# Gongzihang6/Pointcept-KeypointDetection

Hardware: AMD Instinct MI355X
Metric: Mpoints/sec PTv3 fwd @100k pts/scene, 1024-pt window; keypoint offset L2 vs ref (higher is better)
Workload: dtype bf16; 1 GPU; OffsetKeypointPTv3 (PT-v3m1 fork config, 46.2M params) eval forward, 1 x 100000-point synthetic surface scene(s) per GPU, patch 1024, serialization + sparse conv + attention + head included; points_per_gpu=100000, parallelism=replicas x1 (scene-sharded, no collective), forwards_in_flight=1

## Files before the change

### include/ptv3_hip.h

```cpp
#ifndef PTV3_HIP_H
#define PTV3_HIP_H
#include <stddef.h>
#include <stdint.h>

#ifdef __cplusplus
extern "C" {
#endif

#define PTV3_F32 0
#define PTV3_BF16 1

#define PTV3_OK 0
#define PTV3_ERR_ARG 1
#define PTV3_ERR_LAUNCH 2
#define PTV3_ERR_UNSUPPORTED 3

#define PTV3_ORDER_Z 0
#define PTV3_ORDER_Z_TRANS 1
#define PTV3_ORDER_HILBERT 2
#define PTV3_ORDER_HILBERT_TRANS 3

#define PTV3_ACT_NONE 0
#define PTV3_ACT_GELU 1
#define PTV3_ACT_RELU 2
// ... 125 lines not shown
                         const void* res, void* y, const float* gamma2, const float* beta2, void* y2, int64_t m, int c,
                         float eps, int dtype, void* stream);

int ptv3_affine_act(const void* x, const float* scale, const float* shift, int act, void* y, int64_t m,
                    int c, int dtype, void* stream);

int ptv3_cast(const void* x, int src_dtype, void* y, int dst_dtype, int64_t count, void* stream);

size_t ptv3_pool_workspace_bytes(int64_t n);
int ptv3_pool_segments(const int64_t* code0, const int64_t* order0, int64_t n, int shift_bits,
                       const int64_t* batch, int64_t* cluster, int32_t* seg_start, int32_t* n_out,
                       int64_t* pooled_offset, void* workspace, size_t workspace_bytes, void* stream);
int ptv3_pool_reduce(const void* feat, const float* coord, const int64_t* grid_coord,
                     const int64_t* batch, const int64_t* code, int k, const int64_t* order0,
                     const int32_t* seg_start, int64_t n, int64_t n_out, int c, int pooling_depth,
                     const float* bn_scale, const float* bn_shift, int act, const int* row_perm_host,
                     void* feat_out, float* coord_out, int64_t* grid_out, int64_t* batch_out,
                     int64_t* code_out, int dtype, void* stream);

typedef struct {
  int32_t dtype, in_channels , num_stages, num_orders;
  int32_t enc_depths[8], enc_channels[8], enc_heads[8], enc_patch[8];
  int32_t dec_depths[8], dec_channels[8], dec_heads[8], dec_patch[8];
  int32_t stride[8];
  int32_t enc_mode, enable_flash;
  int32_t head_hidden, head_out;
  float mlp_ratio, ln_eps, qk_scale ;
} ptv3_model_desc;

typedef struct {
  const void* grid_coord; int32_t coord_is_i64;
  const void* feat;
  const int64_t* batch;
  const int64_t* offset;
  const int64_t* offset_host;
  int32_t b; int64_t n;
  int32_t depth;
  const int32_t* order_ids_host;
  const int32_t* pool_perm_host;
  int64_t *code, *order, *inverse;
  void* out_feat;
  float* out_head;
  int64_t* stage_points_host;
  int32_t* depth_out;
  int64_t* batch_out;
  int32_t inputs_resident;
  int32_t overlap_calls;
  const void* raw_feat;
  int32_t raw_feat_channels;
  int32_t raw_feat_dtype;
  int64_t arena_n;
  int32_t arena_b;
  void* executor;
} ptv3_forward_io;

void* ptv3_executor_create(void);
int ptv3_executor_destroy(void* executor);

size_t ptv3_forward_workspace_bytes(const ptv3_model_desc* desc, int64_t n, int b);
int ptv3_forward(const ptv3_model_desc* desc, const void* const* params, int num_params,
                 const ptv3_forward_io* io, void* workspace, size_t workspace_bytes, void* stream);

size_t ptv3_gemm_tn_workspace_bytes(int64_t m, int cout, int cin, int kvol);
int ptv3_gemm_tn(const void* dy, const void* x, const int32_t* nbr, float* dw, float* dbias, int64_t m, int cout,
                 int cin, int kvol, int dtype, void* workspace, size_t workspace_bytes, void* stream);
size_t ptv3_col_reduce_workspace_bytes(int64_t m, int c);
int ptv3_col_reduce(const void* a, const void* b, const float* mu, const float* rs, float mu_scale, int mode, float* out,
                    int64_t m, int c, int dtype, void* workspace, size_t workspace_bytes, void* stream);
int ptv3_bn_finalize(const float* sum, const float* centred_sq, int64_t m, const float* weight, const float* bias,
                     float* running_mean, float* running_var, float momentum, float eps, float* mean, float* rstd,
                     float* scale, float* shift, int c, void* stream);
int ptv3_bn_bwd_coeffs(const float* sums, int64_t m, const float* weight, const float* rstd, const float* mean, float* ca,
                       float* cb, float* cc, int c, void* stream);
int ptv3_layernorm_bwd(const void* x, const void* dy, const void* add, const float* gamma, float eps, void* dx,
                       float* dgamma_dbeta, int64_t m, int c, int dtype, void* workspace,
                       size_t workspace_bytes, void* stream);
int ptv3_act_bwd(const void* dy, const void* x, const float* scale, const float* shift, int act, void* dx,
                 int64_t m, int c, int dtype, void* stream);
int ptv3_affine2(const void* dy, const void* x, const float* ca, const float* cb, const float* cc, void* dx,
                 int64_t m, int c, int dtype, void* stream);
int ptv3_pool_max_bwd(const void* feat, const void* dy, const int64_t* order0, const int32_t* seg_start,
                      int64_t n_out, int c, void* dfeat, int dtype, void* stream);
int ptv3_segment_sum(const void* dy, const int64_t* order0, const int32_t* seg_start, int64_t n_out, int c,
                     void* out, int dtype, void* stream);
size_t ptv3_window_attn_bwd_workspace_bytes(int64_t n, int64_t n_pad, int c, int heads, int dtype);
int ptv3_window_attn_bwd(const void* qkv, const void* out, const void* dout, const int32_t* win_order,
                         const int32_t* win_inverse, void* dqkv, int64_t n, int64_t n_pad, int c, int heads,
                         int patch, float scale, int dtype, void* workspace, size_t workspace_bytes,
                         void* stream);
int ptv3_window_attn_varlen_bwd(const void* qkv, const void* out, const void* dout, const int32_t* win_order,
                                const int32_t* win_inverse, const int32_t* cu_seqlens, int num_windows, void* dqkv,
                                int64_t n, int64_t n_pad, int c, int heads, int max_seqlen, float scale, int dtype,
                                void* workspace, size_t workspace_bytes, void* stream);
int ptv3_window_attn_train_fwd(const void* qkv, const int32_t* win_order, const int32_t* win_inverse,
                               const int32_t* cu_seqlens, int num_windows, void* out, float* lse, int64_t n,
                               int64_t n_pad, int c, int heads, int patch, float scale, double sum_len_sq, int dtype,
                               void* stream);
int ptv3_window_attn_train_bwd(const void* qkv, const void* out, const void* dout, const float* lse,
                               const int32_t* win_order, const int32_t* win_inverse, const int32_t* cu_seqlens,
                               int num_windows, void* dqkv, int64_t n, int64_t n_pad, int c, int heads, int patch,
                               float scale, int dtype, void* workspace, size_t workspace_bytes, void* stream);
int ptv3_window_attn_drop_fwd(const void* qkv, const int32_t* win_order, const int32_t* win_inverse,
                              const int32_t* cu_seqlens, int num_windows, void* out, int64_t n, int64_t n_pad, int c,
                              int heads, int patch, float scale, float p_drop, uint32_t seed, int dtype, void* stream);
int ptv3_window_attn_drop_bwd(const void* qkv, const void* out, const void* dout, const int32_t* win_order,
                              const int32_t* win_inverse, const int32_t* cu_seqlens, int num_windows, void* dqkv,
// ... 337 lines not shown
```

### pointcept-keypointdetection_amd/csrc/engine.hip

```cpp
#include <algorithm>
#include <chrono>
#include <mutex>
#include <stdio.h>
#include <stdlib.h>
#include <vector>
#include "common.h"
#include "window_attn.h"

namespace ptv3 {

struct Arena {
  char* base; size_t cap; size_t off; size_t peak; bool dry; bool failed;
  void* alloc(size_t bytes) {
    size_t a = (off + 255) / 256 * 256;
    off = a + bytes;
    if (off > peak) peak = off;
    if (dry) return (void*)(uintptr_t)256;
    if (off > cap) { failed = true; return nullptr; }
    return base + a;
  }
};

__global__ void make_indices_kernel(const int64_t* __restrict__ batch, const void* __restrict__ grid,
                                    int is_i64, int64_t n, int32_t* __restrict__ idx,
// ... 237 lines not shown
    RUN(ptv3_halo_plan_build(L.nbr3, L.row_order, L.n, L.halo, L.halo_bytes, sg));
    if (!dry && ok()) { L.halo_ready = X->event_at(40 + st); (void)hipEventRecord(L.halo_ready, sg); }
  }

  void conv3(Level& L, const void* w, void* out, int C, const float* bias, bool first_block) {
    if (L.halo && !first_block && ptv3_conv_halo_policy(L.n, C, C, 27, d->dtype)) {
      if (!dry && ok() && !L.halo_waited) { (void)hipStreamWaitEvent(sf, L.halo_ready, 0); L.halo_waited = true; }
      RUN(ptv3_conv_halo(L.conv_feat, w, out, L.n, C, L.nbr3, L.row_order, L.halo, L.halo_bytes, bias, nullptr, nullptr, 0,
                         nullptr, nullptr, nullptr, d->dtype, sf));
      return;
    }
    gemm(L.conv_feat, w, out, L.n, C, C, 27, L.nbr3, L.row_order, bias, nullptr, nullptr, 0, nullptr, nullptr, nullptr);
  }

  bool rows_path(int64_t n, int C, int hidden) const {
    static const int64_t min_rows = [] { const char* e = getenv("PTV3_ROWS_MIN"); return e ? atoll(e) : (int64_t)0; }();
    return n >= min_rows && ptv3_rows_linear_capable(C, 3 * C, d->dtype, n) && ptv3_rows_linear_capable(C, C, d->dtype, n) &&
           ptv3_rows_linear_capable(C, hidden, d->dtype, n);
  }

  int patch_K(const Level& L, int patch) const {
    if (d->enable_flash) return patch;
    int64_t mn = L.off_host[0];
    for (size_t i = 1; i < L.off_host.size(); ++i) mn = std::min(mn, L.off_host[i] - L.off_host[i - 1]);
    return (int)std::min<int64_t>(mn, patch);
  }

  void window_plan(Level& L, Plan& P, int K) {
    int64_t n_pad = 0, prev = 0;
    for (int64_t o : L.off_host) {
      int64_t cnt = o - prev;
      n_pad += cnt > K ? (cnt + K - 1) / K * K : cnt;
      prev = o;
    }
    P.K = K; P.n_pad = n_pad;
    bool ragged = false;
    P.nwin = 0; P.sum_len_sq = 0.0; prev = 0;
    for (int64_t o : L.off_host) {
      const int64_t cnt = o - prev;
      prev = o;
      P.nwin += (int)((cnt + K - 1) / K);
      if (cnt < K) { ragged = true; P.sum_len_sq += (double)cnt * cnt; }
      else P.sum_len_sq += (double)((cnt + K - 1) / K) * K * K;
    }
    const int k = d->num_orders;
    int32_t* wo = (int32_t*)G->alloc((size_t)k * n_pad * 4);
    int32_t* wi = (int32_t*)G->alloc((size_t)k * L.n * 4);
    P.cu = (ragged || (dry && d->enable_flash)) ? (int32_t*)G->alloc(((size_t)P.nwin + L.off_host.size() + 1) * 4) : nullptr;
    if (!ragged && !dry) P.cu = nullptr;
    RUN(ptv3_window_plan(L.order, L.inverse, L.offset, (int)L.off_host.size(), k, L.n, n_pad, K, wo, wi, P.cu, sg));
    for (int i = 0; i < k; ++i) { P.wo[i] = wo + (int64_t)i * n_pad; P.wi[i] = wi + (int64_t)i * L.n; }
  }

  hipEvent_t stem_ready = nullptr;
  void level0_sites(Level& L, const void* grid_in, int is_i64) {
    L.indices = (int32_t*)G->alloc((size_t)L.n * 16);
    L.row_order = (int32_t*)G->alloc((size_t)L.n * 4);
    int64_t* g64 = (int64_t*)G->alloc((size_t)L.n * 24);
    L.grid = g64;
    L.table_bytes = ptv3_subm_block_table_bytes(L.n);
    L.table = G->alloc(L.table_bytes);
    RUN(ptv3_subm_sites(L.batch, grid_in, is_i64, L.n, L.indices, g64, L.table, L.table_bytes, sg));
    RUN(ptv3_subm_build_block_table_zeroed(L.indices, L.n, L.table, L.table_bytes, sg));
    if (!dry && ok()) { stem_ready = X->event_at(19); (void)hipEventRecord(stem_ready, sg); }
  }

  void level_tables(Level& L, int st) {
    L.nbr3 = (int32_t*)G->alloc((size_t)L.n * 27 * 4);
    RUN(ptv3_subm_neighbors_blocks(L.indices, L.n, L.table, L.table_bytes, 3, L.nbr3, sg));
    const int Ke = patch_K(L, d->enc_patch[st]);
    window_plan(L, L.plan[0], Ke);
    if (!d->enc_mode && st < d->num_stages - 1) {
      const int Kd = patch_K(L, d->dec_patch[st]);
      if (Kd == Ke) L.plan[1] = L.plan[0]; else window_plan(L, L.plan[1], Kd);
    }
  }

  void level_geometry(Level& L, int st, const void* grid_in, int is_i64) {
    L.indices = (int32_t*)G->alloc((size_t)L.n * 16);
    L.row_order = (int32_t*)G->alloc((size_t)L.n * 4);
    if (!dry && ok())
      hipLaunchKernelGGL(make_indices_kernel, dim3((unsigned)cdiv(L.n, 256)), dim3(256), 0, sg, L.batch, grid_in, is_i64,
                         L.n, L.indices, (int64_t*)nullptr, L.row_order, L.order);
    L.table_bytes = ptv3_subm_block_table_bytes(L.n);
    L.table = G->alloc(L.table_bytes);
    RUN(ptv3_subm_build_block_table(L.indices, L.n, L.table, L.table_bytes, sg));
    level_tables(L, st);
  }

  void attention(const Level& L, const Plan& P, const void* qkv, void* out, int C, int H, int oi, float scale) {
    WindowAttnCall a = window_attn_call(qkv, P.wo[oi], P.wi[oi], out, L.n, P.n_pad, C, H, P.K, scale, d->dtype, sf);
    a.cu_seqlens = P.cu; a.num_windows = P.nwin; a.sum_len_sq = P.sum_len_sq;
    RUN(window_attn_forward(a, {"window_attn", WA_RAGGED_OPTIONAL}));
  }

  void block(Level& L, const Plan& P, int C, int H, int oi, bool first = false) {
    const void* conv_w = next(); const float* conv_b = (const float*)next();
    const float* ln0_g = (const float*)next(); const float* ln0_b = (const float*)next();
    const float* n1_g = (const float*)next(); const float* n1_b = (const float*)next();
    const void* qkv_w = next(); const float* qkv_b = (const float*)next();
    const void* proj_w = next(); const float* proj_b = (const float*)next();
    const float* n2_g = (const float*)next(); const float* n2_b = (const float*)next();
    const void* fc1_w = next(); const float* fc1_b = (const float*)next();
    const void* fc2_w = next(); const float* fc2_b = (const float*)next();
    const int hidden = (int)(C * d->mlp_ratio);
    const size_t mark = F->off;
    const size_t row = (size_t)L.n * es;
    const float scale = d->qk_scale > 0.f ? d->qk_scale : 1.0f / sqrtf((float)(C / H));
    if (ptv3_block_fusable(C, hidden, d->dtype, L.n)) {
      void* f1 = F->alloc(row * C); void* qkv = F->alloc(row * 3 * C); void* t4 = F->alloc(row * C);
      const int splits = ptv3_gemm_splits(L.n, C, C, 27, d->dtype);
      if (L.halo && !first && ptv3_conv_head_halo_policy(L.n, C, d->dtype)) {
        if (!dry && ok() && !L.halo_waited) { (void)hipStreamWaitEvent(sf, L.halo_ready, 0); L.halo_waited = true; }
        RUN(ptv3_conv_head_halo(L.conv_feat, conv_w, conv_b, L.n, C, L.nbr3, L.row_order, L.halo, L.halo_bytes, L.feat,
                                ln0_g, ln0_b, n1_g, n1_b, qkv_w, qkv_b, f1, qkv, d->ln_eps, d->dtype, sf));
      } else if (splits > 1) {
        const size_t wsb = ptv3_gemm_workspace_bytes(L.n, C, C, 27, d->dtype);
        float* slab = (float*)F->alloc(wsb);
        RUN(ptv3_gemm(L.conv_feat, conv_w, nullptr, L.n, C, C, 27, L.nbr3, L.row_order, nullptr, nullptr, nullptr, 0,
                      nullptr, nullptr, nullptr, d->dtype, slab, wsb, sf));
        RUN(ptv3_block_head(nullptr, slab, splits, conv_b, L.feat, ln0_g, ln0_b, n1_g, n1_b, qkv_w, qkv_b, f1, qkv, L.n,
                            C, d->ln_eps, d->dtype, sf));
// ... 15 lines not shown
                            d->ln_eps, d->dtype, sf));
      }
    } else {
      void* t2 = F->alloc(row * C); void* f1 = F->alloc(row * C); void* t3 = F->alloc(row * C);
      void* qkv = F->alloc(row * 3 * C); void* t4 = F->alloc(row * C);
      const int tail_groups = ptv3_block_tail_sliced_policy(C, hidden, d->dtype, L.n);
      const size_t tail_wsb = tail_groups ? ptv3_block_tail_sliced_workspace_bytes(L.n, C, tail_groups) : 0;
      void* tail_ws = tail_wsb ? F->alloc(tail_wsb) : nullptr;
      void* f2 = tail_groups ? nullptr : F->alloc(row * C);
      void* t5 = tail_groups ? nullptr : F->alloc(row * C);
      void* t6 = tail_groups ? nullptr : F->alloc(row * hidden);
      const int splits = ptv3_gemm_splits(L.n, C, C, 27, d->dtype);
      const bool rows = rows_path(L.n, C, hidden);
      if (splits > 1) {
        const size_t wsb = ptv3_gemm_workspace_bytes(L.n, C, C, 27, d->dtype);
        float* slab = (float*)F->alloc(wsb);
        RUN(ptv3_gemm(L.conv_feat, conv_w, nullptr, L.n, C, C, 27, L.nbr3, L.row_order, nullptr, nullptr, nullptr, 0,
                      nullptr, nullptr, nullptr, d->dtype, slab, wsb, sf));
        RUN(ptv3_layernorm_slabs(slab, splits, conv_b, ln0_g, ln0_b, L.feat, f1, n1_g, n1_b, t3, L.n, C, d->ln_eps,
                                 d->dtype, sf));
        gemm(t3, qkv_w, qkv, L.n, C, 3 * C, 1, nullptr, nullptr, qkv_b, nullptr, nullptr, 0, nullptr, nullptr, nullptr);
      } else if (rows) {
        conv3(L, conv_w, t2, C, conv_b, first);
        RUN(ptv3_rows_linear(t2, L.feat, ln0_g, ln0_b, n1_g, n1_b, qkv_w, qkv_b, 0, nullptr, f1, qkv, L.n, C, 3 * C,
                             d->ln_eps, d->dtype, sf));
      } else {
        conv3(L, conv_w, t2, C, conv_b, first);
        RUN(ptv3_layernorm(t2, ln0_g, ln0_b, L.feat, f1, n1_g, n1_b, t3, L.n, C, d->ln_eps, d->dtype, sf));
        gemm(t3, qkv_w, qkv, L.n, C, 3 * C, 1, nullptr, nullptr, qkv_b, nullptr, nullptr, 0, nullptr, nullptr, nullptr);
      }
      attention(L, P, qkv, t4, C, H, oi, scale);
      if (tail_groups) {
        RUN(ptv3_block_tail_sliced(t4, f1, proj_w, proj_b, n2_g, n2_b, fc1_w, fc1_b, fc2_w, fc2_b, L.feat, L.n, C, hidden,
                                   d->ln_eps, d->dtype, tail_groups, tail_ws, tail_wsb, sf));
      } else if (rows) {
        RUN(ptv3_rows_linear(t4, nullptr, nullptr, nullptr, nullptr, nullptr, proj_w, proj_b, 0, f1, nullptr, f2, L.n, C, C,
                             d->ln_eps, d->dtype, sf));
        RUN(ptv3_rows_linear(f2, nullptr, nullptr, nullptr, n2_g, n2_b, fc1_w, fc1_b, PTV3_ACT_GELU, nullptr, nullptr, t6,
                             L.n, C, hidden, d->ln_eps, d->dtype, sf));
      } else {
        gemm(t4, proj_w, f2, L.n, C, C, 1, nullptr, nullptr, proj_b, nullptr, nullptr, 0, f1, nullptr, nullptr);
        RUN(ptv3_layernorm(f2, n2_g, n2_b, nullptr, t5, nullptr, nullptr, nullptr, L.n, C, d->ln_eps, d->dtype, sf));
        gemm(t5, fc1_w, t6, L.n, C, hidden, 1, nullptr, nullptr, fc1_b, nullptr, nullptr, PTV3_ACT_GELU, nullptr, nullptr, nullptr);
      }
      if (!tail_groups)
        gemm(t6, fc2_w, L.feat, L.n, hidden, C, 1, nullptr, nullptr, fc2_b, nullptr, nullptr, 0, f2, nullptr, nullptr);
    }
    L.conv_feat = L.feat;
    F->off = mark;
  }
};

#define RUNR(call) do { if (!dry && R.ok()) { int r__ = (call); if (r__) R.rc = r__; } } while (0)

static int run_forward(Exec* X, const ptv3_model_desc* d, const void* const* params, const ptv3_forward_io* io, Arena& G,
                       Arena& F, hipStream_t sf, bool dry, int* param_count = nullptr) {
  Run R; R.X = X; R.d = d; R.params = params; R.G = &G; R.F = &F; R.sf = sf; R.dry = dry;
  R.es = dtype_bytes(d->dtype);
  const int S = d->num_stages, k = d->num_orders, es = R.es;
  if (!dry) {
    if (!X->geo) {
      X->geo = device_stream(X->device, 0);
      if (!X->geo) {
        set_error("forward: cannot create the geometry stream");
        return PTV3_ERR_LAUNCH;
      }
    }
    if (!io->inputs_resident) {
      hipEvent_t e = X->event_at(0);
      (void)hipEventRecord(e, sf);
      (void)hipStreamWaitEvent(X->geo, e, 0);
    } else {
      (void)hipStreamWaitEvent(X->geo, X->event_at(20 + (X->call & 1)), 0);
    }
  }
  R.sg = dry ? nullptr : X->geo;
  hipStream_t sg = R.sg;
  std::vector<Level> lv(S);
  const int nbits = io->b > 1 ? 32 - __builtin_clz((unsigned)(io->b - 1)) : 0;

  Level& L0 = lv[0];
  L0.n = io->n; L0.batch = io->batch; L0.offset = io->offset;
  L0.code = io->code; L0.order = io->order; L0.inverse = io->inverse;
  L0.off_host.resize(io->b);
  int depth = io->depth;
  const int* hmax = nullptr; const int64_t* hoff = nullptr;
  hipEvent_t read_back = nullptr;
  if (dry) {
    for (int i = 0; i < io->b; ++i) L0.off_host[i] = io->offset_host ? io->offset_host[i] : io->n * (i + 1) / io->b;
    if (depth <= 0) depth = 16;
  } else {
    if (io->offset_host) std::copy(io->offset_host, io->offset_host + io->b, L0.off_host.begin());
    if (depth <= 0 || !io->offset_host) {
      char* pin = (char*)X->pinned_at_least(8 + (size_t)io->b * 8);
      if (!pin) { set_error("forward: cannot allocate the pinned read-back buffer"); return PTV3_ERR_LAUNCH; }
      if (!io->offset_host) hoff = (const int64_t*)(pin + 8);
      if (depth <= 0) {
        int* state = X->coord_max_state();
        if (!state) { set_error("forward: cannot allocate the coordinate-maximum state"); return PTV3_ERR_LAUNCH; }
        hmax = (const int*)pin;
        coord_max(io->grid_coord, io->coord_is_i64, io->n, state, (int*)pin, io->offset, hoff ? io->b : 0,
                  (int64_t*)(pin + 8), sg);
      } else {
        (void)hipMemcpyAsync(pin + 8, io->offset, (size_t)io->b * 8, hipMemcpyDeviceToHost, sg);
      }
      read_back = X->event_at(18);
      (void)hipEventRecord(read_back, sg);
    }
  }
  if (io->batch == nullptr) {
    int64_t* bt = io->batch_out ? io->batch_out : (int64_t*)G.alloc((size_t)io->n * 8);
    if (!dry && R.ok())
      hipLaunchKernelGGL(batch_from_offset_kernel, dim3((unsigned)cdiv(io->n, 256)), dim3(256), 0, sg, io->offset, io->b,
                         io->n, bt);
    L0.batch = bt;
  }
  R.level0_sites(L0, io->grid_coord, io->coord_is_i64);
  const void* stem_w = R.next(); const float* stem_s = (const float*)R.next(); const float* stem_t = (const float*)R.next();
  {
    if (!dry && R.ok()) (void)hipStreamWaitEvent(sf, R.stem_ready, 0);
    const int C0 = d->enc_channels[0];
    L0.feat = F.alloc((size_t)L0.n * C0 * es); L0.channels = C0;
    const void* feat_in = io->feat;
    if (io->raw_feat) {
      void* padded = F.alloc((size_t)L0.n * d->in_channels * es);
      if (!dry && R.ok())
        pad_cast(io->raw_feat, io->raw_feat_dtype, io->raw_feat_channels, padded, d->dtype, d->in_channels, L0.n, sf);
      feat_in = padded;
    }
    RUNR(ptv3_stem_conv_blocks(feat_in, stem_w, L0.feat, L0.n, d->in_channels, C0, 5, L0.indices, L0.table, L0.table_bytes,
                               nullptr, nullptr, stem_s, stem_t, PTV3_ACT_GELU, d->dtype, sf));
    L0.conv_feat = L0.feat;
  }
  if (!dry) {
    if (read_back && X->timed_event_sync(read_back) != hipSuccess) {
      set_error("forward: input read-back failed");
      return PTV3_ERR_LAUNCH;
    }
    if (hoff) std::copy(hoff, hoff + io->b, L0.off_host.begin());
    if (hmax) { depth = 0; for (unsigned v = (unsigned)*hmax + 1; v; v >>= 1) ++depth; }
    PTV3_REQUIRE(depth >= 1 && depth <= 16, "forward: serialization depth %d outside [1,16] (structure.py:81)", depth);
    for (int i = 0; i < io->b; ++i)
      PTV3_REQUIRE(L0.off_host[i] > (i ? L0.off_host[i - 1] : 0), "forward: empty scene %d", i);
    PTV3_REQUIRE(L0.off_host[io->b - 1] == io->n, "forward: offset does not end at n");
  }
  L0.depth = depth;
  if (io->depth_out) *io->depth_out = depth;
  {
    RUNR(ptv3_sfc_encode(io->grid_coord, io->coord_is_i64, L0.batch, io->n, depth, io->order_ids_host, k, L0.code, sg));
    size_t wsb = ptv3_argsort_workspace_bytes(k, io->n);
    void* ws = G.alloc(wsb);
    RUNR(ptv3_argsort_i64_rows(L0.code, k, io->n, std::max(1, 3 * depth + nbits), L0.order, L0.inverse, L0.row_order, ws, wsb,
                               sg));
  }
  R.level_tables(L0, 0);
  if (io->stage_points_host) io->stage_points_host[0] = L0.n;
  if (!dry && R.ok()) { L0.ready = X->event_at(1); (void)hipEventRecord(L0.ready, sg); }
  R.halo_plan(L0, 0);

  auto wait_level = [&](Level& L) { if (!dry && R.ok()) (void)hipStreamWaitEvent(sf, L.ready, 0); };
  struct PoolParams { const void* w; const float *b, *bns, *bnt; };
  wait_level(L0);
  for (int st = 0; st < S; ++st) {
    Level& L = lv[st];
    if (st > 0) {
      Level& P = lv[st - 1];
      PoolParams pp;
      pp.w = R.next(); pp.b = (const float*)R.next(); pp.bns = (const float*)R.next(); pp.bnt = (const float*)R.next();
      const int C = d->enc_channels[st], Cp = d->enc_channels[st - 1];
      int pd = 0; { int v = d->stride[st - 1] - 1; while (v > 0) { ++pd; v >>= 1; } }
      if (pd > P.depth) pd = 0;
      P.cluster = (int64_t*)G.alloc((size_t)P.n * 8);
      P.seg = (int32_t*)G.alloc((size_t)(P.n + 1) * 4);
      int64_t* poff = (int64_t*)G.alloc((size_t)io->b * 8);
      int32_t* nout_dev = (int32_t*)G.alloc(256);
      size_t pwsb = ptv3_pool_workspace_bytes(P.n);
      void* pws = G.alloc(pwsb);
      RUNR(ptv3_pool_segments(P.code, P.order, P.n, 3 * pd, P.batch, P.cluster, P.seg, nout_dev, poff, pws, pwsb, sg));
      L.off_host.resize(io->b);
      if (dry) {
        L.off_host = P.off_host;
      } else if (R.ok()) {
        if (hipMemcpyAsync(L.off_host.data(), poff, (size_t)io->b * 8, hipMemcpyDeviceToHost, sg) != hipSuccess ||
            X->timed_sync(sg) != hipSuccess) { set_error("forward: offset read-back failed"); return PTV3_ERR_LAUNCH; }
      }
      if (!R.ok()) break;
      L.n = L.off_host[io->b - 1]; L.depth = P.depth - pd; L.offset = poff; L.channels = C;
      if (io->stage_points_host) io->stage_points_host[st] = L.n;
      const int* perm = io->pool_perm_host + (size_t)(st - 1) * k;
      int64_t* g = (int64_t*)G.alloc((size_t)L.n * 24);
      int64_t* bt = (int64_t*)G.alloc((size_t)L.n * 8);
      L.code = (int64_t*)G.alloc((size_t)k * L.n * 8);
      L.order = (int64_t*)G.alloc((size_t)k * L.n * 8);
      L.inverse = (int64_t*)G.alloc((size_t)k * L.n * 8);
      RUNR(ptv3_pool_reduce(nullptr, nullptr, P.grid, P.batch, P.code, k, P.order, P.seg, P.n, L.n, C, pd, nullptr,
                           nullptr, 0, perm, nullptr, nullptr, g, bt, L.code, d->dtype, sg));
      L.grid = g; L.batch = bt;
      {
        size_t wsb = ptv3_argsort_workspace_bytes(k, L.n);
        void* ws = G.alloc(wsb);
        RUNR(ptv3_argsort_i64(L.code, k, L.n, std::max(1, 3 * L.depth + nbits), L.order, L.inverse, ws, wsb, sg));
      }
      R.level_geometry(L, st, L.grid, 1);
      if (!d->enc_mode) {
        P.cluster32 = (int32_t*)G.alloc((size_t)P.n * 4);
        if (!dry && R.ok())
          hipLaunchKernelGGL(i64_to_i32_kernel, dim3((unsigned)cdiv(P.n, 256)), dim3(256), 0, sg, P.cluster, P.cluster32, P.n);
      }
      if (!dry && R.ok()) { L.ready = X->event_at(1 + st); (void)hipEventRecord(L.ready, sg); }
      R.halo_plan(L, st);
// ... 14 lines not shown
  if (!d->enc_mode && R.ok()) {
    for (int st = S - 2; st >= 0; --st) {
      Level& P = lv[st];
      Level& Ch = lv[st + 1];
      const int Cd = d->dec_channels[st];
      const int Cin = Ch.channels, Cskip = d->enc_channels[st];
      const void* w = R.next(); const float* b = (const float*)R.next();
      const float* bns = (const float*)R.next(); const float* bnt = (const float*)R.next();
      const void* ws_ = R.next(); const float* bs = (const float*)R.next();
      const float* bnss = (const float*)R.next(); const float* bnst = (const float*)R.next();
      void* skip = F.alloc((size_t)P.n * Cd * es);
      void* fused = (st == 0 && io->out_feat) ? io->out_feat : F.alloc((size_t)P.n * Cd * es);
      const size_t mark = F.off;
      void* up = F.alloc((size_t)Ch.n * Cd * es);
      R.gemm(Ch.feat, w, up, Ch.n, Cin, Cd, 1, nullptr, nullptr, b, bns, bnt, PTV3_ACT_GELU, nullptr, nullptr, nullptr);
      R.gemm(P.feat, ws_, skip, P.n, Cskip, Cd, 1, nullptr, nullptr, bs, bnss, bnst, PTV3_ACT_GELU, up, P.cluster32, fused);
      F.off = mark;
      P.feat = fused; P.conv_feat = skip; P.channels = Cd;
      for (int i = 0; i < d->dec_depths[st]; ++i)
        R.block(P, P.plan[1], Cd, d->dec_heads[st], i % k);
      if (!R.ok()) break;
    }
  }
  if (R.ok() && d->head_out > 0 && !d->enc_mode) {
    Level& L = lv[0];
    const void* w0 = R.next(); const float* b0 = (const float*)R.next();
    const float* bns = (const float*)R.next(); const float* bnt = (const float*)R.next();
    const void* w1 = R.next(); const float* b1 = (const float*)R.next();
    const size_t mark = F.off;
    if (ptv3_mlp2_fusable(L.channels, d->head_hidden, d->head_out, d->dtype)) {
      if (!dry && R.ok()) {
        int r = ptv3_mlp2(L.feat, w0, b0, bns, bnt, PTV3_ACT_RELU, w1, b1, io->out_head, 1, L.n, L.channels,
                          d->head_hidden, d->head_out, d->dtype, sf);
        if (r) R.rc = r;
      }
    } else {
    void* hid = F.alloc((size_t)L.n * d->head_hidden * es);
    R.gemm(L.feat, w0, hid, L.n, L.channels, d->head_hidden, 1, nullptr, nullptr, b0, bns, bnt, PTV3_ACT_RELU, nullptr,
           nullptr, nullptr);
    if (d->dtype == PTV3_F32) {
      R.gemm(hid, w1, io->out_head, L.n, d->head_hidden, d->head_out, 1, nullptr, nullptr, b1, nullptr, nullptr, 0,
             nullptr, nullptr, nullptr);
    } else {
      void* o = F.alloc((size_t)L.n * d->head_out * es);
      R.gemm(hid, w1, o, L.n, d->head_hidden, d->head_out, 1, nullptr, nullptr, b1, nullptr, nullptr, 0, nullptr,
             nullptr, nullptr);
      if (!dry && R.ok()) { int r = ptv3_cast(o, PTV3_BF16, io->out_head, PTV3_F32, L.n * d->head_out, sf); if (r) R.rc = r; }
    }
    }
    F.off = mark;
  }
  if (!dry && R.ok() && !d->enc_mode && io->out_feat && lv[0].feat != io->out_feat)
    (void)hipMemcpyAsync(io->out_feat, lv[0].feat, (size_t)lv[0].n * lv[0].channels * es, hipMemcpyDeviceToDevice, sf);
  if (!dry) (void)hipEventRecord(X->event_at(20 + (X->call & 1)), sf);
  if (param_count) *param_count = R.pi;
  if (G.failed || F.failed) { set_error("forward: workspace arena too small"); return PTV3_ERR_ARG; }
  if (R.rc) return R.rc;
  if (!dry) PTV3_LAUNCH_CHECK();
  return PTV3_OK;
}

static int check_desc(const ptv3_model_desc* d) {
  PTV3_REQUIRE(d->num_stages >= 1 && d->num_stages <= 8, "forward: num_stages %d", d->num_stages);
  PTV3_REQUIRE(d->num_orders >= 1 && d->num_orders <= 8, "forward: num_orders %d", d->num_orders);
  PTV3_REQUIRE(d->dtype == PTV3_F32 || d->dtype == PTV3_BF16, "forward: dtype");
  PTV3_REQUIRE(d->mlp_ratio > 0.f, "forward: mlp_ratio");
  return PTV3_OK;
}

static void plan_bytes(const ptv3_model_desc* desc, int64_t n, int b, size_t* geo, size_t* feat, int* count) {
  std::vector<int> ids(desc->num_orders, 0), perm((size_t)desc->num_stages * desc->num_orders, 0);
  ptv3_forward_io io{};
  io.n = n; io.b = b; io.depth = 0; io.order_ids_host = ids.data(); io.pool_perm_host = perm.data();
  io.coord_is_i64 = 1;
  Arena G{nullptr, 0, 0, 0, true, false}, F{nullptr, 0, 0, 0, true, false};
  run_forward(nullptr, desc, nullptr, &io, G, F, nullptr, true, count);
  *geo = (G.peak + (size_t)b * 16384 * 64 + (1 << 20) + 255) / 256 * 256;
  *feat = (F.peak + (1 << 20) + 255) / 256 * 256;
}

}

using namespace ptv3;

extern "C" int ptv3_coord_max(const void* grid_coord, int coord_is_i64, int64_t n, int32_t* state, int32_t* out_max,
                              void* stream) {
  PTV3_REQUIRE(n >= 1 && n < ((int64_t)1 << 31) && grid_coord && state && out_max, "coord_max: n=%lld or a null pointer",
               (long long)n);
  coord_max(grid_coord, coord_is_i64, n, state, out_max, nullptr, 0, nullptr, (hipStream_t)stream);
  PTV3_LAUNCH_CHECK();
  return PTV3_OK;
}

extern "C" size_t ptv3_forward_workspace_bytes(const ptv3_model_desc* desc, int64_t n, int b) {
  if (check_desc(desc)) return 0;
  size_t g, f;
  plan_bytes(desc, n, b, &g, &f, nullptr);
  return 2 * g + 2 * f + 512;
}

extern "C" void* ptv3_executor_create(void) {
  Exec* X = new Exec();
  (void)hipGetDevice(&X->device);
  return X;
}

extern "C" int ptv3_executor_destroy(void* executor) {
  Exec* X = (Exec*)executor;
  if (!X) return PTV3_OK;
  {
    std::lock_guard<std::mutex> guard(X->mu);
    X->release();
  }
  delete X;
  return PTV3_OK;
}

extern "C" int ptv3_forward(const ptv3_model_desc* desc, const void* const* params, int num_params,
                            const ptv3_forward_io* io, void* workspace, size_t workspace_bytes, void* stream) {
  Exec* X = io->executor ? (Exec*)io->executor : default_exec();
  std::lock_guard<std::mutex> guard(X->mu);
  int cur_dev = 0;
  (void)hipGetDevice(&cur_dev);
  PTV3_REQUIRE(cur_dev == X->device, "forward: executor belongs to device %d, the current device is %d", X->device, cur_dev);
  if (int r = check_desc(desc)) return r;
  PTV3_REQUIRE(io->n >= 1 && io->b >= 1, "forward: empty batch");
  PTV3_REQUIRE(io->depth <= 16, "forward: depth %d > 16", io->depth);
  PTV3_REQUIRE(io->code && io->order && io->inverse, "forward: level-0 serialization outputs are required");
  size_t g, f;
  int count = 0;
  plan_bytes(desc, io->n, io->b, &g, &f, &count);
  PTV3_REQUIRE(count == num_params, "forward: %d parameter pointers given, the model description needs %d",
               num_params, count);
  const bool overlap = io->overlap_calls != 0;
  PTV3_REQUIRE(!overlap || io->inputs_resident, "forward: overlap_calls needs inputs_resident");
  PTV3_REQUIRE(io->raw_feat == nullptr || (io->raw_feat_channels >= 1 && io->raw_feat_channels <= desc->in_channels &&
                                           (io->raw_feat_dtype == PTV3_F32 || io->raw_feat_dtype == PTV3_BF16)),
               "forward: bad raw_feat description");
  if (io->arena_n > 0) {
    PTV3_REQUIRE(io->arena_n >= io->n && io->arena_b >= io->b, "forward: arena capacity (%lld, %d) below this call (%lld, %d)",
                 (long long)io->arena_n, io->arena_b, (long long)io->n, io->b);
    size_t gc, fc;
    plan_bytes(desc, io->arena_n, io->arena_b, &gc, &fc, nullptr);
    PTV3_REQUIRE(gc >= g && fc >= f, "forward: arena capacity plan smaller than this call's plan");
    g = gc; f = fc;
  } else {
    PTV3_REQUIRE(!io->inputs_resident || !overlap, "forward: overlap_calls needs a fixed arena layout (arena_n / arena_b)");
  }
  const size_t need = 2 * g + (overlap ? 2 : 1) * f + 256;
  PTV3_REQUIRE(workspace_bytes >= need, "forward: workspace %zu bytes < %zu (ptv3_forward_workspace_bytes)",
               workspace_bytes, need);
  char* base = (char*)workspace;
  size_t goff = (256 - ((uintptr_t)base & 255)) & 255;
  ++X->call;
  static const bool timing = getenv("PTV3_ENGINE_TIMING") != nullptr;
  const double t_begin = timing ? now_us() : 0.0;
  X->sync_us = 0.0;
  X->event_at(21);
  const unsigned par = X->call & 1;
  hipStream_t caller = (hipStream_t)stream, sf = caller;
  if (overlap) {
    if (!X->feat[par]) X->feat[par] = device_stream(X->device, 1 + par);
    if (!X->feat[par]) {
      set_error("forward: cannot create the feature stream");
      return PTV3_ERR_LAUNCH;
    }
    sf = X->feat[par];
    X->event_at(34);
    if (!X->last_overlap) {
      (void)hipEventRecord(X->event_at(34), caller);
      for (int q = 0; q < 2; ++q)
        if (X->feat[q]) (void)hipStreamWaitEvent(X->feat[q], X->event_at(34), 0);
    }
    (void)hipStreamWaitEvent(sf, X->event_at(30 + (par ^ 1)), 0);
    (void)hipEventRecord(X->event_at(30 + par), caller);
  }
  X->last_overlap = overlap;
  Arena G{base + goff + par * g, g, 0, 0, false, false};
  Arena F{base + goff + 2 * g + (overlap ? par * f : 0), f, 0, 0, false, false};
  int rc = run_forward(X, desc, params, io, G, F, sf, false, nullptr);
  if (overlap) {
    (void)hipEventRecord(X->event_at(32 + par), sf);
    (void)hipStreamWaitEvent(caller, X->event_at(32 + par), 0);
  }
  if (timing)
    fprintf(stderr, "[ptv3_forward] host %.0f us total, %.0f us blocked in read-backs\n", now_us() - t_begin, X->sync_us);
  return rc;
}
// ... 1 lines not shown
```

### pointcept-keypointdetection_amd/pointcept/models/point_transformer_v3/point_transformer_v3m1_base.py

```python
import math
from functools import partial

import torch
import torch.nn as nn

from ptv3_hip import ops
from ptv3_hip import autograd as A
from ptv3_hip import engine as _engine
from pointcept.models.builder import MODELS
from pointcept.models.utils.misc import offset2bincount
from pointcept.models.utils.structure import Point
from pointcept.models.utils.sparse import SubMConv3d, _ParamCache
from pointcept.models.utils.hip_layers import (Linear, LayerNorm, BatchNorm1d, GELU, DropPath, _no_training,
                                                check_sync_batchnorm)
from pointcept.models.modules import PointModule, PointSequential
from pointcept.models.point_prompt_training.prompt_driven_normalization import PDNorm, resolve_norm


RESOLVE_PDNORM = True


class RPE(nn.Module):

    def __init__(self, patch_size, num_heads):
# ... 580 lines not shown


def _input_feat(feat, dtype):
    if feat.dtype not in (torch.float32, torch.bfloat16):
        feat = feat.float()
    feat = feat.contiguous()
    return feat if dtype is None else ops.cast(feat, dtype)


@MODELS.register_module("PT-v3m1")
class PointTransformerV3(PointModule):
    def __init__(
        self,
        in_channels=6,
        order=("z", "z-trans"),
        stride=(2, 2, 2, 2),
        enc_depths=(2, 2, 2, 6, 2),
        enc_channels=(32, 64, 128, 256, 512),
        enc_num_head=(2, 4, 8, 16, 32),
        enc_patch_size=(48, 48, 48, 48, 48),
        dec_depths=(2, 2, 2, 2),
        dec_channels=(64, 64, 128, 256),
        dec_num_head=(4, 4, 8, 16),
        dec_patch_size=(48, 48, 48, 48),
        mlp_ratio=4,
        qkv_bias=True,
        qk_scale=None,
        attn_drop=0.0,
        proj_drop=0.0,
        drop_path=0.3,
        pre_norm=True,
        shuffle_orders=True,
        enable_rpe=False,
        enable_flash=True,
        upcast_attention=False,
        upcast_softmax=False,
        enc_mode=False,
        pdnorm_bn=False,
        pdnorm_ln=False,
        pdnorm_decouple=True,
        pdnorm_adaptive=False,
        pdnorm_affine=True,
        pdnorm_conditions=("ScanNet", "S3DIS", "Structured3D"),
    ):
        super().__init__()
        self.num_stages = len(enc_depths)
        self.order = [order] if isinstance(order, str) else order
        self.enc_mode = enc_mode
        self.shuffle_orders = shuffle_orders
        self.compute_dtype = None
        self.use_engine = True
        self.inputs_resident = False
        self.overlap_calls = False

        assert self.num_stages == len(stride) + 1
        assert self.num_stages == len(enc_depths)
        assert self.num_stages == len(enc_channels)
        assert self.num_stages == len(enc_num_head)
        assert self.num_stages == len(enc_patch_size)
        assert self.enc_mode or self.num_stages == len(dec_depths) + 1
        assert self.enc_mode or self.num_stages == len(dec_channels) + 1
        assert self.enc_mode or self.num_stages == len(dec_num_head) + 1
        assert self.enc_mode or self.num_stages == len(dec_patch_size) + 1

        if (pdnorm_bn or pdnorm_ln) and not pdnorm_decouple:
            raise ValueError("PT-v3m1: pdnorm_decouple=False cannot run in the reference (PDNorm keeps the norm's "
                             "constructor instead of a norm and calls it on the features)")
        if pdnorm_bn:
            bn_layer = partial(PDNorm, norm_layer=partial(BatchNorm1d, eps=1e-3, momentum=0.01, affine=pdnorm_affine),
                               conditions=pdnorm_conditions, decouple=pdnorm_decouple, adaptive=pdnorm_adaptive)
        else:
            bn_layer = partial(BatchNorm1d, eps=1e-3, momentum=0.01)
        if pdnorm_ln:
            ln_layer = partial(PDNorm, norm_layer=partial(LayerNorm, elementwise_affine=pdnorm_affine),
                               conditions=pdnorm_conditions, decouple=pdnorm_decouple, adaptive=pdnorm_adaptive)
        else:
            ln_layer = LayerNorm
        act_layer = GELU

        self.embedding = Embedding(in_channels=in_channels, embed_channels=enc_channels[0], norm_layer=bn_layer,
                                   act_layer=act_layer)

        enc_drop_path = [x.item() for x in torch.linspace(0, drop_path, sum(enc_depths))]
        self.enc = PointSequential()
        for s in range(self.num_stages):
            enc_drop_path_ = enc_drop_path[sum(enc_depths[:s]): sum(enc_depths[: s + 1])]
            enc = PointSequential()
            if s > 0:
                enc.add(SerializedPooling(in_channels=enc_channels[s - 1], out_channels=enc_channels[s],
                                          stride=stride[s - 1], norm_layer=bn_layer, act_layer=act_layer,
                                          shuffle_orders=True), name="down")
            for i in range(enc_depths[s]):
                enc.add(Block(channels=enc_channels[s], num_heads=enc_num_head[s], patch_size=enc_patch_size[s],
                              mlp_ratio=mlp_ratio, qkv_bias=qkv_bias, qk_scale=qk_scale, attn_drop=attn_drop,
                              proj_drop=proj_drop, drop_path=enc_drop_path_[i], norm_layer=ln_layer,
                              act_layer=act_layer, pre_norm=pre_norm, order_index=i % len(self.order),
                              cpe_indice_key=f"stage{s}", enable_rpe=enable_rpe, enable_flash=enable_flash,
                              upcast_attention=upcast_attention, upcast_softmax=upcast_softmax),
                        name=f"block{i}")
            if len(enc) != 0:
                self.enc.add(module=enc, name=f"enc{s}")

        if not self.enc_mode:
            dec_drop_path = [x.item() for x in torch.linspace(0, drop_path, sum(dec_depths))]
            self.dec = PointSequential()
            dec_channels = list(dec_channels) + [enc_channels[-1]]
# ... 77 lines not shown
```

### pointcept-keypointdetection_amd/ptv3_hip/engine.py

```python
import ctypes
from ctypes import addressof, c_int32, c_int64, c_void_p

import torch

from .lib import lib, PTV3_F32, PTV3_BF16, ORDER_IDS, ptv3_model_desc, ptv3_forward_io
from . import ops


class Executor:

    def __init__(self):
        self._dll = lib.load()
        self.handle = self._dll.ptv3_executor_create()
        if not self.handle:
            raise RuntimeError("ptv3_executor_create failed")

    def __deepcopy__(self, memo):
        return Executor()

    def __reduce__(self):
        return (Executor, ())

    def __del__(self):
        try:
# ... 210 lines not shown
            def gen():
                return dict(code=torch.empty(k * cap_n, dtype=torch.int64, device=dev),
                            order=torch.empty(k * cap_n, dtype=torch.int64, device=dev),
                            inverse=torch.empty(k * cap_n, dtype=torch.int64, device=dev),
                            batch=torch.empty(cap_n, dtype=torch.int64, device=dev),
                            out_feat=torch.empty(cap_n * c_out, dtype=dtype, device=dev),
                            out_head=(torch.empty(cap_n * c_head, dtype=torch.float32, device=dev)
                                      if head is not None else None))
            torch.cuda.synchronize(dev)
            backbone.__dict__["_engine_out_ring"] = None
            ring = {"key": rkey, "cap": cap_n, "i": 0, "bufs": [gen() for _ in range(3)]}
            backbone.__dict__["_engine_out_ring"] = ring
            torch.cuda.synchronize(dev)
        cur = ring["bufs"][ring["i"] % 3]
        ring["i"] += 1
        code, order, inverse = (cur[q][:k * n].view(k, n) for q in ("code", "order", "inverse"))
        out_feat = cur["out_feat"][:n * c_out].view(n, c_out)
        out_head = cur["out_head"][:n * c_head].view(n, c_head) if head is not None else None
        if derive_batch:
            batch = cur["batch"][:n]
            point["batch"] = batch
        converted = [t for t, src in ((gc, point.grid_coord), (offset, point.offset)) if t is not src]
        if not derive_batch and batch is not point.batch:
            converted.append(batch)
        if converted:
            torch.cuda.current_stream().synchronize()
        cur["keep"] = (gc, offset, batch, raw)
    else:
        code = torch.empty((k, n), dtype=torch.int64, device=dev)
        order = torch.empty_like(code)
        inverse = torch.empty_like(code)
        out_feat = torch.empty((n, desc.dec_channels[0]), dtype=dtype, device=dev)
        out_head = torch.empty((n, desc.head_out), dtype=torch.float32, device=dev) if head is not None else None
    arena = backbone.__dict__.get("_engine_arena")
    cap = backbone.__dict__.get("_engine_arena_cap", (0, 0, None, None))
    if arena is None or cap[0] < n or cap[1] < nb or cap[2] != dtype or cap[3] != dev:
        cap = (max(n, int(cap[0] * 1.25)), max(nb, cap[1]), dtype, dev)
        ws_bytes = dll.ptv3_forward_workspace_bytes(ctypes.byref(desc), cap[0], cap[1])
        torch.cuda.synchronize(dev)
        backbone.__dict__["_engine_arena"] = None
        arena = torch.empty(ws_bytes, dtype=torch.uint8, device=dev)
        torch.cuda.synchronize(dev)
        backbone.__dict__["_engine_arena"], backbone.__dict__["_engine_arena_cap"] = arena, cap
    execs = backbone.__dict__.setdefault("_engine_exec", {})
    if dev not in execs:
        with torch.cuda.device(dev):
            execs[dev] = Executor()
    stage_pts = (c_int64 * 8)()
    io = ptv3_forward_io()
    io.executor = execs[dev].handle
    io.grid_coord, io.coord_is_i64 = gc.data_ptr(), int(gc.dtype == torch.int64)
    io.feat, io.offset = feat.data_ptr(), offset.data_ptr()
    io.overlap_calls = int(overlap)
    io.arena_n, io.arena_b = cap[0], cap[1]
    if raw is not None:
        io.raw_feat, io.raw_feat_channels = raw.data_ptr(), raw.shape[1]
        io.raw_feat_dtype = PTV3_F32 if raw.dtype == torch.float32 else PTV3_BF16
    else:
        io.raw_feat = None
    if derive_batch:
        io.batch, io.batch_out = None, batch.data_ptr()
        del point["_batch_pending"]
    else:
        io.batch, io.batch_out = batch.data_ptr(), None
    depth_out = c_int32(0)
    io.offset_host, io.b, io.n, io.depth = None, nb, n, 0
    io.depth_out = addressof(depth_out)
    io.inputs_resident = int(bool(getattr(backbone, "inputs_resident", False)))
    io.order_ids_host, io.pool_perm_host = addressof(order_ids), addressof(perm_arr)
    io.code, io.order, io.inverse = code.data_ptr(), order.data_ptr(), inverse.data_ptr()
    io.out_feat = out_feat.data_ptr()
    io.out_head = out_head.data_ptr() if out_head is not None else None
    io.stage_points_host = addressof(stage_pts)
    rc = dll.ptv3_forward(ctypes.byref(desc), pk.table, len(pk.tensors), ctypes.byref(io), arena.data_ptr(),
                          arena.numel(), ops._stream())
    lib.check(rc, "ptv3_forward")
    depth = int(depth_out.value)
    assert depth * 3 + nb.bit_length() <= 63
    point["order"] = list(backbone.order)
    point["serialized_depth"] = depth
    point["serialized_code"], point["serialized_order"], point["serialized_inverse"] = code, order, inverse
    point["feat"] = out_feat
    point["_stage_points"] = [int(stage_pts[i]) for i in range(S)]
    return point, out_head
```

Baseline: 45.80 Mpoints/s.

## Fork level-0 site/table build onto feature stream to overlap with host readback

Adds a lead_in_order mode that, by default, runs batch derivation, level-0 site extraction and block-table build on the feature stream instead of the geometry stream. The stem conv is deferred until after the host offset readback and validation, so it can overlap with SFC encoding and argsort on the geometry stream. Cross-stream events are added to hand the batch and table to the geometry stream, plus a final join. The fork is skipped when the previous call is still in flight. This adds event and ordering complexity and the risk of cross-stream races.

```diff
diff --git a/include/ptv3_hip.h b/include/ptv3_hip.h
--- a/include/ptv3_hip.h
+++ b/include/ptv3_hip.h
@@ -201,6 +201,7 @@
   int64_t arena_n;
   int32_t arena_b;
   void* executor;
+  int32_t lead_in_order;
 } ptv3_forward_io;
 
 void* ptv3_executor_create(void);
diff --git a/pointcept-keypointdetection_amd/csrc/engine.hip b/pointcept-keypointdetection_amd/csrc/engine.hip
--- a/pointcept-keypointdetection_amd/csrc/engine.hip
+++ b/pointcept-keypointdetection_amd/csrc/engine.hip
@@ -313,22 +313,28 @@
     for (int i = 0; i < k; ++i) { P.wo[i] = wo + (int64_t)i * n_pad; P.wi[i] = wi + (int64_t)i * L.n; }
   }
 
-  hipEvent_t stem_ready = nullptr;
-  void level0_sites(Level& L, const void* grid_in, int is_i64) {
+  hipEvent_t table_ready = nullptr;
+  void level0_sites(Level& L, const void* grid_in, int is_i64, hipStream_t s) {
     L.indices = (int32_t*)G->alloc((size_t)L.n * 16);
     L.row_order = (int32_t*)G->alloc((size_t)L.n * 4);
     int64_t* g64 = (int64_t*)G->alloc((size_t)L.n * 24);
     L.grid = g64;
     L.table_bytes = ptv3_subm_block_table_bytes(L.n);
     L.table = G->alloc(L.table_bytes);
-    RUN(ptv3_subm_sites(L.batch, grid_in, is_i64, L.n, L.indices, g64, L.table, L.table_bytes, sg));
-    RUN(ptv3_subm_build_block_table_zeroed(L.indices, L.n, L.table, L.table_bytes, sg));
-    if (!dry && ok()) { stem_ready = X->event_at(19); (void)hipEventRecord(stem_ready, sg); }
+    RUN(ptv3_subm_sites(L.batch, grid_in, is_i64, L.n, L.indices, g64, L.table, L.table_bytes, s));
+  }
+  void level0_table(Level& L, hipStream_t s) {
+    RUN(ptv3_subm_build_block_table_zeroed(L.indices, L.n, L.table, L.table_bytes, s));
+    if (!dry && ok()) { table_ready = X->event_at(19); (void)hipEventRecord(table_ready, s); }
+  }
+
+  void neighbors3(Level& L, hipStream_t s) {
+    L.nbr3 = (int32_t*)G->alloc((size_t)L.n * 27 * 4);
+    RUN(ptv3_subm_neighbors_blocks(L.indices, L.n, L.table, L.table_bytes, 3, L.nbr3, s));
   }
 
   void level_tables(Level& L, int st) {
-    L.nbr3 = (int32_t*)G->alloc((size_t)L.n * 27 * 4);
-    RUN(ptv3_subm_neighbors_blocks(L.indices, L.n, L.table, L.table_bytes, 3, L.nbr3, sg));
+    if (!L.nbr3) neighbors3(L, sg);
     const int Ke = patch_K(L, d->enc_patch[st]);
     window_plan(L, L.plan[0], Ke);
     if (!d->enc_mode && st < d->num_stages - 1) {
@@ -450,6 +456,9 @@
 };
 
 #define RUNR(call) do { if (!dry && R.ok()) { int r__ = (call); if (r__) R.rc = r__; } } while (0)
+#ifndef PTV3_L0_NBR3_AT
+#define PTV3_L0_NBR3_AT 0
+#endif
 
 static int run_forward(Exec* X, const ptv3_model_desc* d, const void* const* params, const ptv3_forward_io* io, Arena& G,
                        Arena& F, hipStream_t sf, bool dry, int* param_count = nullptr) {
@@ -474,6 +483,17 @@
   }
   R.sg = dry ? nullptr : X->geo;
   hipStream_t sg = R.sg;
+  bool fork = false;
+  if (!dry) {
+    fork = io->lead_in_order != 1;
+    if (io->lead_in_order == 0 && io->inputs_resident && !io->overlap_calls &&
+        hipEventQuery(X->event_at(20 + ((X->call & 1) ^ 1))) == hipErrorNotReady) {
+      (void)hipGetLastError();
+      fork = false;
+    }
+    if (fork) (void)hipStreamWaitEvent(sf, X->event_at(20 + (X->call & 1)), 0);
+  }
+  hipStream_t sc = fork ? sf : sg;
   std::vector<Level> lv(S);
   const int nbits = io->b > 1 ? 32 - __builtin_clz((unsigned)(io->b - 1)) : 0;
 
@@ -506,17 +526,20 @@
       (void)hipEventRecord(read_back, sg);
     }
   }
+  hipEvent_t batch_ready = nullptr;
   if (io->batch == nullptr) {
     int64_t* bt = io->batch_out ? io->batch_out : (int64_t*)G.alloc((size_t)io->n * 8);
-    if (!dry && R.ok())
-      hipLaunchKernelGGL(batch_from_offset_kernel, dim3((unsigned)cdiv(io->n, 256)), dim3(256), 0, sg, io->offset, io->b,
+    if (!dry && R.ok()) {
+      hipLaunchKernelGGL(batch_from_offset_kernel, dim3((unsigned)cdiv(io->n, 256)), dim3(256), 0, sc, io->offset, io->b,
                          io->n, bt);
+      if (fork) { batch_ready = X->event_at(17); (void)hipEventRecord(batch_ready, sf); }
+    }
     L0.batch = bt;
   }
-  R.level0_sites(L0, io->grid_coord, io->coord_is_i64);
+  R.level0_sites(L0, io->grid_coord, io->coord_is_i64, sc);
   const void* stem_w = R.next(); const float* stem_s = (const float*)R.next(); const float* stem_t = (const float*)R.next();
-  {
-    if (!dry && R.ok()) (void)hipStreamWaitEvent(sf, R.stem_ready, 0);
+  auto stem = [&]() {
+    if (!fork && !dry && R.ok()) (void)hipStreamWaitEvent(sf, R.table_ready, 0);
     const int C0 = d->enc_channels[0];
     L0.feat = F.alloc((size_t)L0.n * C0 * es); L0.channels = C0;
     const void* feat_in = io->feat;
@@ -529,7 +552,15 @@
     RUNR(ptv3_stem_conv_blocks(feat_in, stem_w, L0.feat, L0.n, d->in_channels, C0, 5, L0.indices, L0.table, L0.table_bytes,
                                nullptr, nullptr, stem_s, stem_t, PTV3_ACT_GELU, d->dtype, sf));
     L0.conv_feat = L0.feat;
-  }
+#if PTV3_L0_NBR3_AT == 2
+    if (fork) {
+      R.neighbors3(L0, sf);
+      if (!dry && R.ok()) (void)hipEventRecord(R.table_ready, sf);
+    }
+#endif
+  };
+  R.level0_table(L0, sc);
+  if (!fork) stem();
   if (!dry) {
     if (read_back && X->timed_event_sync(read_back) != hipSuccess) {
       set_error("forward: input read-back failed");
@@ -537,23 +568,35 @@
     }
     if (hoff) std::copy(hoff, hoff + io->b, L0.off_host.begin());
     if (hmax) { depth = 0; for (unsigned v = (unsigned)*hmax + 1; v; v >>= 1) ++depth; }
-    PTV3_REQUIRE(depth >= 1 && depth <= 16, "forward: serialization depth %d outside [1,16] (structure.py:81)", depth);
-    for (int i = 0; i < io->b; ++i)
-      PTV3_REQUIRE(L0.off_host[i] > (i ? L0.off_host[i - 1] : 0), "forward: empty scene %d", i);
-    PTV3_REQUIRE(L0.off_host[io->b - 1] == io->n, "forward: offset does not end at n");
+    const int bad = [&]() -> int {
+      PTV3_REQUIRE(depth >= 1 && depth <= 16, "forward: serialization depth %d outside [1,16] (structure.py:81)", depth);
+      for (int i = 0; i < io->b; ++i)
+        PTV3_REQUIRE(L0.off_host[i] > (i ? L0.off_host[i - 1] : 0), "forward: empty scene %d", i);
+      PTV3_REQUIRE(L0.off_host[io->b - 1] == io->n, "forward: offset does not end at n");
+      return PTV3_OK;
+    }();
+    if (bad) {
+      if (fork) (void)hipEventRecord(X->event_at(20 + (X->call & 1)), sf);
+      return bad;
+    }
   }
   L0.depth = depth;
   if (io->depth_out) *io->depth_out = depth;
+  if (!dry && R.ok() && batch_ready) (void)hipStreamWaitEvent(sg, batch_ready, 0);
+  RUNR(ptv3_sfc_encode(io->grid_coord, io->coord_is_i64, L0.batch, io->n, depth, io->order_ids_host, k, L0.code, sg));
+  if (fork) stem();
   {
-    RUNR(ptv3_sfc_encode(io->grid_coord, io->coord_is_i64, L0.batch, io->n, depth, io->order_ids_host, k, L0.code, sg));
     size_t wsb = ptv3_argsort_workspace_bytes(k, io->n);
     void* ws = G.alloc(wsb);
     RUNR(ptv3_argsort_i64_rows(L0.code, k, io->n, std::max(1, 3 * depth + nbits), L0.order, L0.inverse, L0.row_order, ws, wsb,
                                sg));
   }
+  const bool nbr3_on_sf = fork && L0.nbr3 != nullptr;
+  if (fork && !nbr3_on_sf && !dry && R.ok()) (void)hipStreamWaitEvent(sg, R.table_ready, 0);
   R.level_tables(L0, 0);
   if (io->stage_points_host) io->stage_points_host[0] = L0.n;
   if (!dry && R.ok()) { L0.ready = X->event_at(1); (void)hipEventRecord(L0.ready, sg); }
+  if (nbr3_on_sf && !dry && R.ok()) (void)hipStreamWaitEvent(sg, R.table_ready, 0);
   R.halo_plan(L0, 0);
 
   auto wait_level = [&](Level& L) { if (!dry && R.ok()) (void)hipStreamWaitEvent(sf, L.ready, 0); };
@@ -674,7 +717,11 @@
   }
   if (!dry && R.ok() && !d->enc_mode && io->out_feat && lv[0].feat != io->out_feat)
     (void)hipMemcpyAsync(io->out_feat, lv[0].feat, (size_t)lv[0].n * lv[0].channels * es, hipMemcpyDeviceToDevice, sf);
-  if (!dry) (void)hipEventRecord(X->event_at(20 + (X->call & 1)), sf);
+  if (!dry) {
+    (void)hipEventRecord(X->event_at(16), sg);
+    (void)hipStreamWaitEvent(sf, X->event_at(16), 0);
+    (void)hipEventRecord(X->event_at(20 + (X->call & 1)), sf);
+  }
   if (param_count) *param_count = R.pi;
   if (G.failed || F.failed) { set_error("forward: workspace arena too small"); return PTV3_ERR_ARG; }
   if (R.rc) return R.rc;
@@ -756,6 +803,8 @@
                num_params, count);
   const bool overlap = io->overlap_calls != 0;
   PTV3_REQUIRE(!overlap || io->inputs_resident, "forward: overlap_calls needs inputs_resident");
+  PTV3_REQUIRE(io->lead_in_order >= 0 && io->lead_in_order <= 2, "forward: lead_in_order %d outside [0,2]",
+               io->lead_in_order);
   PTV3_REQUIRE(io->raw_feat == nullptr || (io->raw_feat_channels >= 1 && io->raw_feat_channels <= desc->in_channels &&
                                            (io->raw_feat_dtype == PTV3_F32 || io->raw_feat_dtype == PTV3_BF16)),
                "forward: bad raw_feat description");
diff --git a/pointcept-keypointdetection_amd/pointcept/models/point_transformer_v3/point_transformer_v3m1_base.py b/pointcept-keypointdetection_amd/pointcept/models/point_transformer_v3/point_transformer_v3m1_base.py
--- a/pointcept-keypointdetection_amd/pointcept/models/point_transformer_v3/point_transformer_v3m1_base.py
+++ b/pointcept-keypointdetection_amd/pointcept/models/point_transformer_v3/point_transformer_v3m1_base.py
@@ -656,6 +656,7 @@
         self.use_engine = True
         self.inputs_resident = False
         self.overlap_calls = False
+        self.lead_in_order = 0
 
         assert self.num_stages == len(stride) + 1
         assert self.num_stages == len(enc_depths)
diff --git a/pointcept-keypointdetection_amd/ptv3_hip/engine.py b/pointcept-keypointdetection_amd/ptv3_hip/engine.py
--- a/pointcept-keypointdetection_amd/ptv3_hip/engine.py
+++ b/pointcept-keypointdetection_amd/ptv3_hip/engine.py
@@ -286,6 +286,7 @@
     io.grid_coord, io.coord_is_i64 = gc.data_ptr(), int(gc.dtype == torch.int64)
     io.feat, io.offset = feat.data_ptr(), offset.data_ptr()
     io.overlap_calls = int(overlap)
+    io.lead_in_order = int(getattr(backbone, "lead_in_order", 0))
     io.arena_n, io.arena_b = cap[0], cap[1]
     if raw is not None:
         io.raw_feat, io.raw_feat_channels = raw.data_ptr(), raw.shape[1]
```

Result: no change. 46.08 Mpoints/s (median of 6 runs) (+0.6%).
